# arkiven4/glow-tts

Hardware: AMD Instinct MI355X
Metric: mel_frames_per_sec_train_step (higher is better)
Workload: dtype bf16; 1 GPU; configs/base.json, LJSpeech-shaped synthetic batches, B=32/GPU, T_x<=150, T_y<=800, bf16 GEMMs; batch_per_gpu=32, T_x=150, T_y=800, batches_rotated=8, padded_frames_per_gpu_step=25600, rows_layout=ragged, graphs_captured=6, parallelism=dp1 (utterance-sharded, RCCL gradient all-reduce, fp32 on the wire), launch=one HIP graph per step (one per ragged-row bucket, captured up front)

## Files before the change

### glow-tts_amd/_lib.py

```python
import ctypes
import os

_HERE = os.path.dirname(os.path.abspath(__file__))
LIB_PATH = os.environ.get("GT_LIB") or os.path.join(_HERE, "libglowtts_hip.so")

c_void_p, c_int, c_i64, c_size_t, c_float, c_u32 = (ctypes.c_void_p, ctypes.c_int, ctypes.c_int64,
                                                    ctypes.c_size_t, ctypes.c_float, ctypes.c_uint32)


class Pointer(ctypes.c_void_p):

    @classmethod
    def from_param(cls, v):
        if hasattr(v, "data_ptr"):
            v = v.data_ptr()
        elif isinstance(v, ctypes.Structure):
            return ctypes.byref(v)
        return ctypes.c_void_p.from_param(v)


STATUS = "status"
c_void_p = Pointer

PROTOTYPES = {
    "gt_version": (ctypes.c_char_p, []),
    "gt_mas_f32": (STATUS, [c_void_p, c_void_p, c_void_p, c_void_p, c_void_p, c_int, c_void_p, c_void_p,
                            c_int, c_int, c_int, c_i64, c_i64, c_void_p, c_size_t, c_void_p, c_void_p]),
    "gt_mas_lds_bytes": (c_size_t, [c_int, c_int]),
    "gt_mas_workspace_bytes": (c_size_t, [c_int, c_int, c_int]),
    "gt_mas_long_f32": (STATUS, [c_void_p, c_void_p, c_void_p, c_void_p, c_void_p, c_int, c_void_p, c_void_p,
                                 c_int, c_int, c_int, c_i64, c_i64, c_void_p, c_size_t, c_void_p, c_void_p]),
    "gt_mas_long_workspace_bytes": (c_size_t, [c_int, c_int, c_int]),
    "gt_mas_lengths_from_mask_f32": (STATUS, [c_void_p, c_void_p, c_void_p, c_int, c_int, c_int,
                                              c_i64, c_i64, c_void_p]),
    "gt_conv_gemm_bf16": (STATUS, [c_void_p, c_int, c_void_p, c_void_p, c_void_p, c_int, c_void_p,
                                   c_void_p, c_int, c_int, c_void_p, c_int, c_void_p, c_void_p, c_int,
                                   c_int, c_int, c_int, c_int, c_int, c_int, c_int,
                                   c_int, c_int, c_float, c_u32, c_void_p, c_void_p, c_int, c_int, c_void_p]),
    "gt_conv_wgrad_workspace_bytes": (c_size_t, [c_int, c_int, c_int, c_int, c_void_p]),
    "gt_conv_wgrad_ci_tile": (c_int, [c_int]),
    "gt_conv_wgrad_bf16": (STATUS, [c_void_p, c_int, c_void_p, c_int, c_int, c_int, c_int, c_int, c_void_p, c_size_t, c_void_p]),
    "gt_weightnorm_bwd": (STATUS, [c_void_p, c_int, c_void_p, c_void_p, c_void_p, c_void_p, c_void_p, c_void_p,
                                   c_int, c_int, c_int, c_int, c_void_p]),
    "gt_conv_wgrad_batched": (STATUS, [c_void_p, c_void_p, c_int, c_int, c_int, c_void_p]),
    "gt_weightnorm_bwd_batched": (STATUS, [c_void_p, c_int, c_int, c_int, c_void_p]),
    "gt_adamw_flat": (STATUS, [c_void_p, c_void_p, c_void_p, c_void_p, c_size_t, c_void_p, c_void_p, c_void_p]),
    "gt_colsum": (STATUS, [c_void_p, c_int, c_int, c_void_p, c_int, c_int, c_void_p]),
    "gt_squeeze_rows_f32": (STATUS, [c_void_p, c_void_p, c_void_p, c_int, c_int, c_int, c_int, c_void_p, c_void_p]),
    "gt_unsqueeze_rows_f32": (STATUS, [c_void_p, c_void_p, c_void_p, c_int, c_int, c_int, c_int, c_void_p, c_void_p]),
    "gt_flow_scalars": (STATUS, [c_void_p, c_int, c_void_p, c_void_p, c_void_p]),
    "gt_flow_scalars_multi": (STATUS, [c_void_p, c_void_p, c_int, c_void_p, c_int, c_void_p]),
    "gt_actnorm_ddi": (STATUS, [c_void_p, c_void_p, c_int, c_int, c_int, c_void_p, c_void_p, c_void_p, c_void_p]),
    "gt_actnorm_invconv_fwd": (STATUS, [c_void_p, c_void_p, c_void_p, c_int, c_void_p, c_void_p, c_void_p, c_void_p,
                                        c_void_p, c_void_p, c_void_p, c_int, c_int, c_int, c_void_p]),
    "gt_actnorm_invconv_bwd": (STATUS, [c_void_p, c_void_p, c_void_p, c_void_p, c_void_p, c_void_p, c_void_p, c_void_p,
                                        c_void_p, c_void_p, c_void_p, c_void_p, c_void_p, c_int, c_int, c_int, c_void_p]),
    "gt_actnorm_invconv_rev": (STATUS, [c_void_p, c_void_p, c_void_p, c_int, c_void_p, c_void_p, c_void_p, c_void_p, c_int, c_int, c_void_p]),
    "gt_coupling_rev": (STATUS, [c_void_p, c_void_p, c_void_p, c_void_p, c_int, c_int, c_int, c_void_p]),
    "gt_coupling_fwd": (STATUS, [c_void_p, c_void_p, c_void_p, c_void_p, c_void_p, c_int, c_int, c_int, c_int, c_void_p, c_int, c_void_p]),
    "gt_coupling_bwd": (STATUS, [c_void_p, c_void_p, c_void_p, c_void_p, c_void_p, c_void_p, c_void_p,
                                 c_int, c_int, c_int, c_int, c_void_p, c_int, c_void_p]),
    "gt_gate_bwd": (STATUS, [c_void_p, c_int, c_void_p, c_void_p, c_int, c_void_p, c_int, c_void_p,
                             c_int, c_int, c_float, c_u32, c_void_p, c_void_p]),
    "gt_relu_drop_bwd": (STATUS, [c_void_p, c_int, c_void_p, c_int, c_void_p, c_int, c_int, c_int, c_float, c_void_p]),
    "gt_rows_add_bf16": (STATUS, [c_void_p, c_int, c_void_p, c_int, c_int, c_int, c_void_p]),
    "gt_rows_f32_to_bf16": (STATUS, [c_void_p, c_int, c_void_p, c_int, c_void_p, c_int, c_int, c_void_p]),
    "gt_layernorm_fwd": (STATUS, [c_void_p, c_void_p, c_int, c_void_p, c_void_p, c_void_p, c_void_p, c_void_p, c_int,
                                  c_void_p, c_void_p, c_int, c_int, c_float, c_float, c_u32, c_float, c_u32, c_int, c_void_p, c_void_p]),
    "gt_layernorm_bwd": (STATUS, [c_void_p, c_void_p, c_int, c_void_p, c_void_p, c_void_p, c_void_p, c_void_p, c_int, c_int,
                                  c_float, c_float, c_u32, c_float, c_u32, c_int, c_void_p, c_void_p, c_void_p, c_int,
                                  c_void_p, c_void_p, c_int, c_void_p, c_void_p, c_void_p]),
    "gt_layernorm_bwd_partial_rows": (c_int, [c_int]),
    "gt_layernorm_bwd_partials": (STATUS, [c_void_p, c_void_p, c_int, c_void_p, c_void_p, c_void_p, c_void_p, c_void_p, c_int, c_int,
                                           c_float, c_float, c_u32, c_float, c_u32, c_int, c_void_p, c_void_p, c_void_p, c_int,
                                           c_void_p, c_void_p, c_int, c_void_p, c_void_p]),
    "gt_param_partials_reduce": (STATUS, [c_void_p, c_void_p]),
    "gt_dds_bwd_partial_rows": (c_int, [c_int]),
    "gt_attn_fwd": (STATUS, [c_void_p, c_void_p, c_void_p, c_int, c_void_p, c_void_p, c_void_p, c_void_p, c_int, c_void_p,
                             c_int, c_int, c_int, c_void_p, c_int, c_int, c_int, c_float, c_u32, c_void_p, c_void_p]),
    "gt_attn_bwd_workspace_bytes": (c_size_t, [c_int, c_int, c_int]),
    "gt_attn_mfma_shape": (c_int, [c_int, c_int, c_int]),
    "gt_attn_long_shape": (c_int, [c_int, c_int, c_int]),
    "gt_attn_bwd": (STATUS, [c_void_p, c_void_p, c_void_p, c_int, c_void_p, c_void_p, c_void_p, c_void_p, c_int, c_void_p,
                             c_void_p, c_size_t, c_void_p, c_void_p, c_void_p, c_int, c_void_p, c_void_p,
                             c_int, c_int, c_int, c_void_p, c_int, c_int, c_int, c_float, c_u32, c_void_p, c_void_p]),
    "gt_attn_stats_bytes": (c_size_t, [c_int, c_int, c_int]),
    "gt_attn_bwd_stats_workspace_bytes": (c_size_t, [c_int, c_int, c_int]),
    "gt_attn_fwd_stats": (STATUS, [c_void_p, c_void_p, c_void_p, c_int, c_void_p, c_void_p, c_void_p, c_void_p, c_int, c_void_p,
                                   c_int, c_int, c_int, c_void_p, c_int, c_int, c_int, c_float, c_u32, c_void_p, c_void_p]),
    "gt_attn_bwd_stats": (STATUS, [c_void_p, c_void_p, c_void_p, c_int, c_void_p, c_void_p, c_void_p, c_void_p, c_int, c_void_p,
                                   c_void_p, c_size_t, c_void_p, c_void_p, c_void_p, c_int, c_void_p, c_void_p,
                                   c_int, c_int, c_int, c_void_p, c_int, c_int, c_int, c_float, c_u32, c_void_p, c_void_p]),
    "gt_embedding_fwd": (STATUS, [c_void_p, c_void_p, c_void_p, c_void_p, c_void_p, c_int, c_int, c_int, c_void_p, c_int, c_int, c_int, c_float, c_void_p]),
    "gt_embedding_bwd": (STATUS, [c_void_p, c_void_p, c_void_p, c_void_p, c_int, c_int, c_int, c_void_p, c_int, c_int, c_int, c_float, c_void_p]),
    "gt_rows_add_cond": (STATUS, [c_void_p, c_int, c_void_p, c_int, c_void_p, c_void_p, c_void_p, c_int, c_void_p, c_int,
                                  c_int, c_int, c_int, c_int, c_void_p, c_void_p]),
    "gt_rows_ctx_fill": (STATUS, [c_void_p, c_void_p, c_void_p, c_void_p, c_void_p, c_void_p, c_int, c_int, c_void_p]),
    "gt_step_inputs": (STATUS, [c_void_p, c_void_p]),
# ... 390 lines not shown
```

### glow-tts_amd/csrc/conv_wgrad.hip

```cpp
#include <stdlib.h>
#include "common.h"
#include "internal.h"
#include "mfma_frag.h"
#include "../../include/glowtts_hip.h"

namespace {

constexpr int SLAB_Q = 64;

typedef __attribute__((__vector_size__(4 * sizeof(short)))) short s16x4_t;

__device__ __forceinline__ unsigned lds_off(const void* p) { return (unsigned)reinterpret_cast<uintptr_t>(p); }

__device__ __forceinline__ bf16x8_t tr_frag(const unsigned char* p0, const unsigned char* p1) {
  const s16x4_t lo = __builtin_amdgcn_ds_read_tr16_b64_v4i16((__attribute__((address_space(3))) s16x4_t*)(uintptr_t)p0);
  const s16x4_t hi = __builtin_amdgcn_ds_read_tr16_b64_v4i16((__attribute__((address_space(3))) s16x4_t*)(uintptr_t)p1);
  typedef __attribute__((__vector_size__(8 * sizeof(short)))) short s16x8_t;
  s16x8_t v = {lo[0], lo[1], lo[2], lo[3], hi[0], hi[1], hi[2], hi[3]};
  return __builtin_bit_cast(bf16x8_t, v);
}

__device__ __forceinline__ void glds16(const void* src, unsigned dst_base) {
  unsigned keep;
  asm volatile("s_mov_b32 %0, m0\n\ts_mov_b32 m0, %2\n\ts_nop 0\n\t"
               "global_load_lds_dwordx4 %1, off\n\ts_mov_b32 m0, %0"
               : "=&s"(keep) : "v"(src), "s"(dst_base) : "memory");
}
template <int N> __device__ __forceinline__ void wait_vm() { asm volatile("s_waitcnt vmcnt(%0)" :: "n"(N) : "memory"); }

template <int TAPS, int NJ, int KB_, int NST_> struct WgGeo {
  static constexpr int KB = KB_, NST = NST_;
  static constexpr int XR = KB + TAPS - 1;
  static constexpr int XCH = 8 * NJ;
  static constexpr int YB = KB * 256, XB = XR * XCH * 16, STAGE = YB + XB;
  static constexpr int YI = KB / 16;
  static constexpr int NWX = XR * XCH / 4;
  static constexpr int XI = (NWX + 63) / 64;
  static constexpr int NLD = YI + XI;
  static constexpr int NB = TAPS * NJ;
  static constexpr int LDS = NST * STAGE;
  static_assert(KB % 16 == 0 && SLAB_Q % KB == 0, "stage rows");
  static_assert((XR * XCH) % 4 == 0, "X chunks split evenly over the waves");
  static_assert(LDS <= 80 * 1024, "two workgroups per CU");
  static_assert((NST - 2) * NLD <= 63, "vmcnt field");
  static_assert(TAPS == 1 || NJ == 1, "taps or channel groups");
};

template <int TAPS, int NJ, int KB_, int NST_>
__device__ __forceinline__ void wgrad_tile(
    const bf16_t* __restrict__ X, int ldx, const bf16_t* __restrict__ dY, int ldy,
    float* __restrict__ part, float* __restrict__ part_bias, int R, int Cin, int Cout, int slab_rows,
    int co0, int ci0, int slab, int co_begin, int Ncols)
{
  using G = WgGeo<TAPS, NJ, KB_, NST_>;
  constexpr int KB = G::KB, NST = G::NST, NB = G::NB;
  extern __shared__ __attribute__((aligned(1024))) unsigned char ring[];
  const int tid = threadIdx.x, lane = tid & 63, wave = __builtin_amdgcn_readfirstlane(tid >> 6);
  constexpr int padl = TAPS >> 1;
  const int mbeg = slab * slab_rows;
  const int mend = min(R, mbeg + slab_rows);
  const int nst = (mend - mbeg + KB - 1) / KB;
  const int wco = wave >> 1, wci = wave & 1;
  const bool do_bias = (ci0 == 0) && part_bias && wci == 0;

  f32x16_t acc[NB][2];
  float bsum[2] = {0.f, 0.f};
#pragma unroll
  for (int t = 0; t < NB; ++t)
#pragma unroll
    for (int j = 0; j < 2; ++j)
#pragma unroll
      for (int e = 0; e < 16; ++e) acc[t][j][e] = 0.0f;

  int yrow[G::YI], ycol[G::YI], xrow[G::XI], xcol[G::XI];
  bool xact[G::XI];
#pragma unroll
  for (int j = 0; j < G::YI; ++j) {
    const int L = j * 256 + tid, r = L >> 4, c = (L & 15) ^ ((r & 3) << 2);
    yrow[j] = r; ycol[j] = min(co0 + c * 8, Ncols - 8);
// ... 114 lines not shown
      const int ci = ci0 + j * 64 + wci * 32 + r;
#pragma unroll
      for (int i = 0; i < 2; ++i) {
        if (ci >= Cin) continue;
#pragma unroll
        for (int e = 0; e < 16; ++e) {
          const int co = co0 + wco * 64 + i * 32 + (e & 3) + 8 * (e >> 2) + 4 * h;
          if (co < Ncols) part[(((size_t)slab * TAPS + t) * Cout + co_begin + co) * Cin + ci] = acc[t * NJ + j][i][e];
        }
      }
    }
  if (do_bias) {
#pragma unroll
    for (int i = 0; i < 2; ++i) {
      const float tot = bsum[i] + __shfl_xor(bsum[i], 32);
      const int co = co0 + wco * 64 + i * 32 + r;
      if (h == 0 && co < Ncols) part_bias[(size_t)slab * Cout + co_begin + co] = tot;
    }
  }
}

template <int TAPS> struct WgSel;
template <> struct WgSel<5> { static constexpr int NJ = 1, KB = 64, NST = 3; };
template <> struct WgSel<3> { static constexpr int NJ = 1, KB = 64, NST = 3; };
template <> struct WgSel<1> { static constexpr int NJ = 3, KB = 32, NST = 3; };
template <int TAPS> using WgGeoT = WgGeo<TAPS, WgSel<TAPS>::NJ, WgSel<TAPS>::KB, WgSel<TAPS>::NST>;

template <int TAPS>
__global__ __launch_bounds__(256, 2) void gt_conv_wgrad_kernel(
    const bf16_t* __restrict__ X, int ldx, const bf16_t* __restrict__ dY, int ldy,
    float* __restrict__ part, float* __restrict__ part_bias, int R, int Cin, int Cout, int slab_rows)
{
  using S = WgSel<TAPS>;
  wgrad_tile<TAPS, S::NJ, S::KB, S::NST>(X, ldx, dY, ldy, part, part_bias, R, Cin, Cout, slab_rows,
                                         blockIdx.x * 128, blockIdx.y * 64 * S::NJ, blockIdx.z, 0, Cout);
}

template <int TAPS>
__global__ __launch_bounds__(256, 2) void gt_conv_wgrad_batched_kernel(
    const gt_wgrad_job* __restrict__ jobs, const gt_wgrad_tile* __restrict__ tiles)
{
  using S = WgSel<TAPS>;
  const gt_wgrad_tile t = tiles[blockIdx.x];
  const gt_wgrad_job j = jobs[t.job];
  wgrad_tile<TAPS, S::NJ, S::KB, S::NST>(static_cast<const bf16_t*>(j.X), j.ldx, static_cast<const bf16_t*>(j.dY), j.ldy,
                                         j.part, j.part_bias, j.R, j.Cin, j.Cout, j.slab_rows, t.co0, t.ci0, t.slab, j.co_begin, j.co_count);
}

template <int TAPS> static int wgrad_lds_attr()
{
  if (gt_allow_lds<&gt_conv_wgrad_kernel<TAPS>>(WgGeoT<TAPS>::LDS) || gt_allow_lds<&gt_conv_wgrad_batched_kernel<TAPS>>(WgGeoT<TAPS>::LDS)) return GT_E_LAUNCH;
  return 0;
}

constexpr int WNB_ROWS = 4;
__device__ __forceinline__ void weightnorm_bwd_row(
    const float* __restrict__ part, const float* __restrict__ part_bias, int S, const float* __restrict__ v,
    const float* __restrict__ g, const float* __restrict__ inv_norm, float* __restrict__ dv, float* __restrict__ dg,
    float* __restrict__ dbias, int Cout, int Cin, int taps, int accumulate, int co, float* dws)
{
  const int lane = threadIdx.x & 63, n = Cin * taps;
  if (dbias && lane == 0) {
    float sb = 0.f;
    for (int k = 0; k < S; ++k) sb += part_bias[(size_t)k * Cout + co];
    dbias[co] = accumulate ? dbias[co] + sb : sb;
  }
  const size_t sstride = (size_t)taps * Cout * Cin;
  for (int tap = 0; tap < taps; ++tap) {
    const float* pt = part + ((size_t)tap * Cout + co) * Cin;
    for (int ci = lane; ci < Cin; ci += 64) {
      const float* pp = pt + ci;
      float s0 = 0.f, s1 = 0.f, s2 = 0.f, s3 = 0.f;
      int k = 0;
      for (; k + 4 <= S; k += 4) {
        const float a0 = pp[(size_t)k * sstride], a1 = pp[(size_t)(k + 1) * sstride];
        const float a2 = pp[(size_t)(k + 2) * sstride], a3 = pp[(size_t)(k + 3) * sstride];
        s0 += a0; s1 += a1; s2 += a2; s3 += a3;
      }
      for (; k < S; ++k) s0 += pp[(size_t)k * sstride];
      dws[ci * taps + tap] = (s0 + s1) + (s2 + s3);
    }
  }
  __builtin_amdgcn_fence(__ATOMIC_RELEASE, "wavefront");
  __builtin_amdgcn_wave_barrier();
  __builtin_amdgcn_fence(__ATOMIC_ACQUIRE, "wavefront");
  const float* vr = v + (size_t)co * n;
  float* dr = dv + (size_t)co * n;
  if (!g) {
    for (int i = lane; i < n; i += 64) dr[i] = accumulate ? dr[i] + dws[i] : dws[i];
    return;
  }
  float dot = 0.f;
  for (int i = lane; i < n; i += 64) dot += dws[i] * vr[i];
  const float d = wave_sum(dot);
  const float inv = inv_norm[co], gg = g[co];
  if (lane == 0) dg[co] = accumulate ? dg[co] + d * inv : d * inv;
  const float a = gg * inv, bcoef = gg * d * inv * inv * inv;
  for (int i = lane; i < n; i += 64) {
    const float val = a * dws[i] - bcoef * vr[i];
    dr[i] = accumulate ? dr[i] + val : val;
  }
}

constexpr int WNF_P = 4;
typedef float wnf4_t __attribute__((ext_vector_type(4)));
__device__ __forceinline__ wnf4_t wnf_ld4(const float* p) { return *(const __attribute__((address_space(1))) wnf4_t*)(uintptr_t)p; }
// ... 244 lines not shown
                                  int taps, void* workspace, size_t workspace_bytes, void* stream)
{
  if (R <= 0 || Cin <= 0 || Cout <= 0) return GT_E_INVAL;
  if (!X || !dY || !workspace) return GT_E_INVAL;
  if (taps != 1 && taps != 3 && taps != 5) return GT_E_UNSUPPORTED;
  if ((Cin & 7) || (Cout & 7) || (ldx & 7) || (ldy & 7)) return GT_E_ALIGN;
  if (((uintptr_t)X | (uintptr_t)dY) & 15) return GT_E_ALIGN;
  int S = 0;
  if (workspace_bytes < gt_conv_wgrad_workspace_bytes(R, Cin, Cout, taps, &S)) return GT_E_INVAL;
  const int slab_rows = (((R + S - 1) / S) + SLAB_Q - 1) / SLAB_Q * SLAB_Q;
  const int cit = gt_conv_wgrad_ci_tile(taps);
  const dim3 grid((Cout + 127) / 128, (Cin + cit - 1) / cit, S);
  hipStream_t st = static_cast<hipStream_t>(stream);
  const bf16_t* x = static_cast<const bf16_t*>(X); const bf16_t* dy = static_cast<const bf16_t*>(dY);
  float* part = static_cast<float*>(workspace);
  float* pb = part + (size_t)S * taps * Cout * Cin;
  if (wgrad_lds_attr<5>() || wgrad_lds_attr<3>() || wgrad_lds_attr<1>()) return GT_E_LAUNCH;
  if (taps == 5)      hipLaunchKernelGGL(gt_conv_wgrad_kernel<5>, grid, dim3(256), WgGeoT<5>::LDS, st, x, ldx, dy, ldy, part, pb, R, Cin, Cout, slab_rows);
  else if (taps == 3) hipLaunchKernelGGL(gt_conv_wgrad_kernel<3>, grid, dim3(256), WgGeoT<3>::LDS, st, x, ldx, dy, ldy, part, pb, R, Cin, Cout, slab_rows);
  else                hipLaunchKernelGGL(gt_conv_wgrad_kernel<1>, grid, dim3(256), WgGeoT<1>::LDS, st, x, ldx, dy, ldy, part, pb, R, Cin, Cout, slab_rows);
  return gt_launch_status(__func__);
}

extern "C" int gt_weightnorm_bwd(const void* workspace, int R, const float* v, const float* g, const float* inv_norm,
                                 float* dv, float* dg, float* dbias, int Cout, int Cin, int taps, int accumulate, void* stream)
{
  if (!workspace || !v || !dv || Cout <= 0 || Cin <= 0 || taps <= 0) return GT_E_INVAL;
  if (g && (!inv_norm || !dg)) return GT_E_INVAL;
  int S = 0;
  gt_conv_wgrad_workspace_bytes(R, Cin, Cout, taps, &S);
  if ((size_t)WNB_ROWS * Cin * taps * sizeof(float) > WNB_LDS_MAX) return GT_E_UNSUPPORTED;
  const int rows = wnb_rows(Cin * taps);
  const size_t lds = wnb_lds(rows, Cin * taps);
  const float* part = static_cast<const float*>(workspace);
  hipLaunchKernelGGL(gt_weightnorm_bwd_kernel, dim3((Cout + rows - 1) / rows), dim3(64 * rows), lds, static_cast<hipStream_t>(stream),
                     part, part + (size_t)S * taps * Cout * Cin, S, v, g, inv_norm, dv, dg, dbias, Cout, Cin, taps, accumulate);
  return gt_launch_status(__func__);
}

extern "C" int gt_conv_wgrad_batched(const void* jobs_device, const void* tiles_device, int n_tiles5, int n_tiles3,
                                     int n_tiles1, void* stream)
{
  if (!jobs_device || !tiles_device || n_tiles5 < 0 || n_tiles3 < 0 || n_tiles1 < 0) return GT_E_INVAL;
  hipStream_t st = static_cast<hipStream_t>(stream);
  const gt_wgrad_job* jobs = static_cast<const gt_wgrad_job*>(jobs_device);
  const gt_wgrad_tile* tiles = static_cast<const gt_wgrad_tile*>(tiles_device);
  if (wgrad_lds_attr<5>() || wgrad_lds_attr<3>() || wgrad_lds_attr<1>()) return GT_E_LAUNCH;
  if (n_tiles5) hipLaunchKernelGGL(gt_conv_wgrad_batched_kernel<5>, dim3(n_tiles5), dim3(256), WgGeoT<5>::LDS, st, jobs, tiles);
  if (n_tiles3) hipLaunchKernelGGL(gt_conv_wgrad_batched_kernel<3>, dim3(n_tiles3), dim3(256), WgGeoT<3>::LDS, st, jobs, tiles + n_tiles5);
  if (n_tiles1) hipLaunchKernelGGL(gt_conv_wgrad_batched_kernel<1>, dim3(n_tiles1), dim3(256), WgGeoT<1>::LDS, st, jobs, tiles + n_tiles5 + n_tiles3);
  return gt_launch_status(__func__);
}

extern "C" int gt_weightnorm_bwd_batched(const void* jobs_device, int n_jobs, int total_rows, int max_row_elems, void* stream)
{
  if (!jobs_device || n_jobs <= 0 || total_rows <= 0 || max_row_elems <= 0) return GT_E_INVAL;
  if ((size_t)WNB_ROWS * max_row_elems * sizeof(float) > WNB_LDS_MAX) return GT_E_UNSUPPORTED;
  const int rows = wnb_rows(max_row_elems);
  const size_t lds = wnb_lds(rows, max_row_elems);
  hipLaunchKernelGGL(gt_weightnorm_bwd_batched_kernel, dim3((total_rows + rows - 1) / rows), dim3(64 * rows), lds,
                     static_cast<hipStream_t>(stream), static_cast<const gt_wnb_job*>(jobs_device), n_jobs, total_rows, max_row_elems);
  return gt_launch_status(__func__);
}

extern "C" int gt_colsum(const void* Y, int ldy, int is_f32, float* out, int R, int N, void* stream)
{
  if (!Y || !out || R < 0 || N <= 0) return GT_E_INVAL;
  if (R == 0) return GT_OK;
  const int rows_per_block = 128;
  const dim3 grid((N + 63) / 64, (R + rows_per_block - 1) / rows_per_block);
  hipStream_t st = static_cast<hipStream_t>(stream);
  if (is_f32) hipLaunchKernelGGL(gt_colsum_kernel<true>,  grid, dim3(256), 0, st, Y, ldy, out, R, N, rows_per_block);
  else        hipLaunchKernelGGL(gt_colsum_kernel<false>, grid, dim3(256), 0, st, Y, ldy, out, R, N, rows_per_block);
  return gt_launch_status(__func__);
}
```

### glow-tts_amd/wgrad.py

```python
import contextlib
import os
import types

import numpy as np
import torch

from . import _lib, devstate
from ._lib import call

JOB = np.dtype([("X", "u8"), ("dY", "u8"), ("part", "u8"), ("part_bias", "u8"), ("ldx", "i4"), ("ldy", "i4"), ("R", "i4"),
                ("Cin", "i4"), ("Cout", "i4"), ("co_begin", "i4"), ("co_count", "i4"), ("slab_rows", "i4")])
TILE = np.dtype([("job", "i4"), ("co0", "i4"), ("ci0", "i4"), ("slab", "i4")])
WNB = np.dtype([("part", "u8"), ("part_bias", "u8"), ("v", "u8"), ("g", "u8"), ("inv_norm", "u8"), ("dv", "u8"), ("dg", "u8"),
                ("dbias", "u8"), ("S", "i4"), ("Cout", "i4"), ("Cin", "i4"), ("taps", "i4"), ("row_start", "i4"),
                ("accumulate", "i4"), ("pad0_", "i4"), ("pad1_", "i4")])
assert JOB.itemsize == 64 and TILE.itemsize == 16 and WNB.itemsize == 96
C_STRUCTS = {"gt_wgrad_job": JOB, "gt_wgrad_tile": TILE, "gt_wnb_job": WNB}

SLOTS = 512
ROW_US = float(os.environ.get("GT_WGRAD_ROW_US", "0.033"))
WG_US = 3.0
PART_BPS = 2.0e6
MAX_SLABS = 32
XCDS = 8
CI_TILE = {5: 64, 3: 64, 1: 192}
FORCE_SLABS = int(os.environ.get("GT_WGRAD_SLABS", "0"))

ASYNC = os.environ.get("GT_WGRAD_ASYNC", "0") != "0"
_ACTIVE = []
_KEEP = []
_SCOPE = None


_POOL = []
_POOL_N, _POOL_BYTES = 64, 1 << 18


def _fill_pool():
    while len(_POOL) < _POOL_N:
        _POOL.append(torch.empty(_POOL_BYTES, dtype=torch.uint8).pin_memory())


class CaptureKeep(list):

    def release(self):
        for obj in self:
            if isinstance(obj, torch.Tensor) and not obj.is_cuda and obj.numel() == _POOL_BYTES and obj.is_pinned() and len(_POOL) < 4 * _POOL_N:
                _POOL.append(obj)
        self.clear()


@contextlib.contextmanager
def capture_scope(dev, nbytes=8 << 20):
    global _SCOPE
    arena = torch.empty(nbytes, dtype=torch.uint8, device=dev)
    sc = _SCOPE = types.SimpleNamespace(dev=dev, arena=arena, off=0, uploads=[], keep=CaptureKeep([arena]))
    try:
        yield sc.keep
        assert not (arena.is_cuda and torch.cuda.is_current_stream_capturing())
        for dst, host in sc.uploads:
            dst.copy_(host, non_blocking=True)
        if sc.uploads and arena.is_cuda:
            torch.cuda.current_stream(dev).synchronize()
    except BaseException:
        sc.keep.release()
        raise
    finally:
        sc.uploads.clear()
        _SCOPE = None


def capture_keep(obj):
    if _SCOPE is not None:
        if not any(o is obj for o in _SCOPE.keep):
            _SCOPE.keep.append(obj)
        return True
    return False


def choose_slabs(base_tiles, R, part_bytes):
    if FORCE_SLABS:
        return FORCE_SLABS
    best, costs = None, []
    for S in range(1, max(1, min(MAX_SLABS, R // 128)) + 1):
        rounds = -(-base_tiles * S // SLOTS)
        rows = -(-(-(-R // S)) // 64) * 64
        cost = rounds * (rows * ROW_US + WG_US) + S * part_bytes / PART_BPS
        costs.append((cost, S))
        best = cost if best is None else min(best, cost)
    return min(S for cost, S in costs if cost <= 1.05 * best)


def single_slabs(R, Cin, Cout, taps):
    import ctypes
    S = ctypes.c_int(0)
    call.gt_conv_wgrad_workspace_bytes(R, Cin, Cout, taps, ctypes.byref(S))
    return S.value


def _side_stream(dev):
    return devstate.get(dev).stream("wgrad_side")


def join(dev):
    st = devstate.get(dev)
    if st.pending:
        torch.cuda.current_stream(dev).wait_stream(st.stream("wgrad_side"))
        st.pending = False


def active():
    return _ACTIVE[-1] if _ACTIVE else None


def _scratch(dev, nbytes):
    return devstate.get(dev).scratch("wgrad_flush", nbytes, per_stream=True)


def _grad_out(param):
    fg = getattr(param, "_gt_flat_grad", None)
    if fg is None:
        return torch.empty_like(param)
    buf, off = fg
    return buf[off:off + param.numel()].view_as(param)


class WgradQueue:

    def __init__(self, device, site=None, accumulate=False, side_stream=False):
        self.dev = device
        self.site = site
        self.items = []
        self.accumulate, self.force_side = accumulate, side_stream
        self.defer_to = None
        self.ln_jobs = []
        self.params_done = []

    def __enter__(self):
        _ACTIVE.append(self)
        return self

    def __exit__(self, et, ev, tb):
        _ACTIVE.pop()
# ... 106 lines not shown
            devstate.get(dev).pending = True
        else:
            self._flush()

    def _keep(self, obj):
        if capture_keep(obj):
            return
        if self.site is not None:
            lst = getattr(self.site, "_wgrad_keep", None)
            if lst is None:
                lst = []
                object.__setattr__(self.site, "_wgrad_keep", lst)
            lst.append(obj)
        else:
            _KEEP.append(obj)

    def _flush(self):
        dev = self.dev
        jobs, tiles, wnbs, rows, max_n, nbytes = self._plan()
        ws = _scratch(dev, nbytes)
        base = ws.data_ptr()
        capturing = torch.cuda.is_current_stream_capturing()

        def upload(arr):
            raw = arr.view(np.uint8).reshape(-1)
            if capturing:
                if not _POOL or raw.size > _POOL_BYTES:
                    raise RuntimeError("wgrad tables: no pinned staging buffer available inside graph capture "
                                       "(run one eager step first)")
                full = _POOL.pop()
                host = full[: raw.size]
                host.numpy()[:] = raw
                self._keep(full)
                sc = _SCOPE
                nb = (raw.size + 255) & ~255
                if sc is not None and sc.dev == dev and sc.off + nb <= sc.arena.numel():
                    dst = sc.arena[sc.off:sc.off + raw.size]
                    sc.off += nb
                    sc.uploads.append((dst, host))
                    return dst
                return host.to(dev, non_blocking=True)
            host = torch.from_numpy(raw).pin_memory()
            return host.to(dev, non_blocking=True)

        if capturing:
            cache = {}
        else:
            _fill_pool()
            cache = getattr(self.site, "_wgrad_tables", None) if self.site is not None else None
            if cache is None:
                cache = {}
                if self.site is not None:
                    object.__setattr__(self.site, "_wgrad_tables", cache)
        skey = tuple((t, tuple(x[2:] for x in tiles[t]), tuple(j[6:] for j in jobs)) for t in (5, 3, 1))
        if cache.get("skey") != skey:
            tl, counts = [], []
            for taps in (5, 3, 1):
                n = 0
                order = sorted(range(len(tiles[taps])), key=lambda i: -tiles[taps][i][0])
                queues = [[] for _ in range(XCDS)]
                for i in order:
                    _, jid, nco, nci, S = tiles[taps][i]
                    for sl in range(S):
                        q = min(queues, key=len)
                        q += [(jid, co * 128, ci * CI_TILE[taps], sl) for co in range(nco) for ci in range(nci)]
                flat = [q[pos] for pos in range(max(map(len, queues), default=0)) for q in queues if pos < len(q)]
                if flat:
                    t = np.zeros(len(flat), dtype=TILE)
                    a = np.array(flat, dtype=np.int64)
                    t["job"], t["co0"], t["ci0"], t["slab"] = a[:, 0], a[:, 1], a[:, 2], a[:, 3]
                    tl.append(t)
                    n = len(flat)
                counts.append(n)
            ta = np.concatenate(tl) if tl else np.zeros(1, dtype=TILE)
            cache["skey"], cache["tiles"], cache["counts"] = skey, upload(ta), counts
            cache["pkey"] = None
        pkey = (base, tuple(j[:4] for j in jobs), tuple(w[2:8] for w in wnbs), self.accumulate)
        if cache.get("pkey") != pkey:
            ja = np.array([(j[0], j[1], base + j[2], (base + j[3]) if j[3] >= 0 else 0) + j[4:] for j in jobs], dtype=JOB)
            wa = np.array([(base + w[0], base + w[1]) + w[2:] for w in wnbs], dtype=WNB)
            cache["pkey"], cache["jobs"], cache["wnb"] = pkey, upload(ja), upload(wa)
        counts = cache["counts"]
        st = _lib.current_stream(dev)
        assert all(call.gt_conv_wgrad_ci_tile(t) == w for t, w in CI_TILE.items()), "wgrad.CI_TILE does not match the library's tile widths"
        call.gt_conv_wgrad_batched(cache["jobs"], cache["tiles"], counts[0], counts[1], counts[2], st)
        call.gt_weightnorm_bwd_batched(cache["wnb"], len(wnbs), rows, max_n, st)
        if capturing:
            self._keep(cache)
        self.items = []
```

### include/glowtts_hip.h

```cpp
#ifndef GLOWTTS_HIP_H
#define GLOWTTS_HIP_H

#include <stddef.h>
#include <stdint.h>

#ifdef __cplusplus
extern "C" {
#endif

#define GT_OK            0
#define GT_E_INVAL      -1
#define GT_E_UNSUPPORTED -2
#define GT_E_ALIGN      -3
#define GT_E_LAUNCH     -4

#define GT_DT_F32  0
#define GT_DT_I32  1
#define GT_DT_F16  2
#define GT_DT_BF16 3
#define GT_DT_U8   4

#define GT_MAS_ST_TX_GT_TY   1
#define GT_MAS_ST_BAD_LEN    2

// ... 26 lines not shown

int gt_mas_lengths_from_mask_f32(const float* mask, int32_t* t_x, int32_t* t_y,
                                 int B, int T_x, int T_y, int64_t stride_b, int64_t stride_x,
                                 void* stream);

#define GT_HALO 2

#define GT_TILE_AUTO 0
#define GT_TILE_64x64 1
#define GT_TILE_64x128 2
#define GT_TILE_128x64 3
#define GT_TILE_128x128 4
#define GT_TILE_256x64 5
#define GT_TILE_64x64_TAPS 6
int gt_conv_gemm_bf16(const void* X, int ldx, const void* Wp, const float* bias,
                      const float* cond, int ldc, const float* rowmask,
                      void* Y, int ldy, int out_f32, const void* addend, int ldadd,
                      void* gate_t, void* gate_s, int ldts,
                      int R, int N, int Cin, int taps, int Tp, int Np, int Kp,
                      int relu, int gate, float drop_p, uint32_t drop_seed, const uint32_t* seed_dev,
                      const int32_t* row0, int B, int tile, void* stream);

int gt_pack_conv_weights(const float* v, const float* g, void* pack_fwd, void* pack_dgrad,
                         float* inv_norm, int Cout, int Cin, int taps,
                         int Np_fwd, int Kp_fwd, int Np_dgrad, int Kp_dgrad, int gate, void* stream);

typedef struct gt_pack_desc {
  const float* v; const float* g; void* pack_fwd; void* pack_dgrad; float* inv_norm;
  int32_t Cout, Cin, taps, Np_fwd, Kp_fwd, Np_dgrad, Kp_dgrad, gate, row_start, pad_;
} gt_pack_desc;
int gt_pack_conv_weights_multi(const void* descs_device, int n_convs, int total_rows, int group8, void* stream);

size_t gt_conv_wgrad_workspace_bytes(int R, int Cin, int Cout, int taps, int* slabs_out);
int gt_conv_wgrad_ci_tile(int taps);
int gt_conv_wgrad_bf16(const void* X, int ldx, const void* dY, int ldy, int R, int Cin, int Cout,
                       int taps, void* workspace, size_t workspace_bytes, void* stream);

int gt_weightnorm_bwd(const void* workspace, int R, const float* v, const float* g, const float* inv_norm,
                      float* dv, float* dg, float* dbias, int Cout, int Cin, int taps, int accumulate, void* stream);

typedef struct gt_wgrad_job {
  const void* X; const void* dY; float* part; float* part_bias;
  int32_t ldx, ldy, R, Cin, Cout, co_begin, co_count, slab_rows;
} gt_wgrad_job;
typedef struct gt_wgrad_tile { int32_t job, co0, ci0, slab; } gt_wgrad_tile;
typedef struct gt_wnb_job {
  const float* part; const float* part_bias; const float* v; const float* g; const float* inv_norm;
  float* dv; float* dg; float* dbias;
  int32_t S, Cout, Cin, taps, row_start, accumulate, pad0_, pad1_;
} gt_wnb_job;
int gt_conv_wgrad_batched(const void* jobs_device, const void* tiles_device, int n_tiles5, int n_tiles3,
                          int n_tiles1, void* stream);
int gt_weightnorm_bwd_batched(const void* jobs_device, int n_jobs, int total_rows, int max_row_elems, void* stream);

int gt_colsum(const void* Y, int ldy, int is_f32, float* out, int R, int N, void* stream);

int gt_squeeze_rows_f32(const float* y, float* rows, const int32_t* len_sq, int B, int C, int Ty, int Tp,
                        const int32_t* row0, void* stream);
int gt_unsqueeze_rows_f32(const float* rows, float* y, const int32_t* len_sq, int B, int C, int Ty, int Tp,
                          const int32_t* row0, void* stream);

int gt_actnorm_ddi(const float* x, const int32_t* len, int B, int R, int C, double* workspace, float* logs, float* bias,
                   void* stream);

int gt_flow_scalars(const float* logs, int C, const float* W, float* scal, void* stream);
int gt_flow_scalars_multi(const void* logs_ptrs, const void* w_ptrs, int C, float* scal, int n, void* stream);
int gt_actnorm_invconv_fwd(const float* x, float* y, void* y0_bf16, int ld0, const float* logs, const float* bias,
                           const float* W, const float* scal, const float* rowmask, const int32_t* len,
                           float* logdet, int B, int R, int C, void* stream);
int gt_actnorm_invconv_bwd(const float* x, const float* dy, float* dx, const float* logs, const float* bias,
                           const float* W, const float* scal, const float* rowmask, const int32_t* len,
                           const float* dlogdet, float* dlogs, float* dbias, float* dW, int B, int R, int C, void* stream);

int gt_coupling_fwd(const float* out, const float* x, float* z, const float* rowmask, float* logdet,
                    int B, int R, int C, int Tp, const int32_t* row0, int sigmoid_scale, void* stream);
int gt_coupling_bwd(const float* out, const float* x, const float* dz, const float* dlogdet, const float* rowmask,
                    float* dx, void* dout_bf16, int B, int R, int C, int Tp, const int32_t* row0, int sigmoid_scale,
                    void* stream);

int gt_gate_bwd(const void* dacts, int ldd, const void* T, const void* S, int ldts, void* dpre, int ldp, void* dpre_cond,
                int R, int half, float drop_p, uint32_t drop_seed, const uint32_t* seed_dev, void* stream);

int gt_relu_drop_bwd(const void* d, int ldd, const void* y, int ldy, void* dc, int ldc, int R, int n, float drop_p, void* stream);

int gt_rows_add_bf16(float* dx, int ldx, const void* add, int lda, int R, int n, void* stream);
int gt_rows_f32_to_bf16(const float* in, int ldi, void* out, int ldo, const float* rowmask, int R, int n, void* stream);

int gt_layernorm_fwd(const float* a, const void* y, int ldy, const float* gamma, const float* beta, const float* rowmask,
                     float* out_f32, void* out_bf16, int ldo, float* mean, float* rstd, int R, int C, float eps,
                     float p_in, uint32_t seed_in, float p_out, uint32_t seed_out, int relu, const uint32_t* seed_dev, void* stream);
int gt_layernorm_bwd(const float* a, const void* y, int ldy, const float* gamma, const float* beta, const float* rowmask,
                     const float* mean, const float* rstd, int R, int C, float eps,
                     float p_in, uint32_t seed_in, float p_out, uint32_t seed_out, int relu, const uint32_t* seed_dev,
                     const float* dout_f32, const void* dout_bf16, int lddo,
                     float* da, void* dy, int lddy, float* dgamma, float* dbeta, void* stream);
int gt_layernorm_bwd_partial_rows(int R);
int gt_layernorm_bwd_partials(const float* a, const void* y, int ldy, const float* gamma, const float* beta, const float* rowmask,
                              const float* mean, const float* rstd, int R, int C, float eps,
                              float p_in, uint32_t seed_in, float p_out, uint32_t seed_out, int relu, const uint32_t* seed_dev,
                              const float* dout_f32, const void* dout_bf16, int lddo,
                              float* da, void* dy, int lddy, float* partials, void* stream);
#define GT_PARTIALS_MAX 32
typedef struct gt_partials_job { const float* partials; float* dst_a; float* dst_b; int32_t n_rows, Ca, Cb, pad_; } gt_partials_job;
typedef struct gt_partials_args { gt_partials_job job[GT_PARTIALS_MAX]; int32_t n_jobs; } gt_partials_args;
int gt_param_partials_reduce(const gt_partials_args* args, void* stream);

// ... 348 lines not shown
```

Baseline: 4.838 million mel-frames/s.

## Add paired 512-thread wgrad kernel sharing dY or X tiles across two output tiles

```diff
diff --git a/glow-tts_amd/_lib.py b/glow-tts_amd/_lib.py
--- a/glow-tts_amd/_lib.py
+++ b/glow-tts_amd/_lib.py
@@ -44,6 +44,7 @@
                                    c_int, c_int, c_int, c_int, c_void_p]),
     "gt_conv_wgrad_batched": (STATUS, [c_void_p, c_void_p, c_int, c_int, c_int, c_void_p]),
     "gt_weightnorm_bwd_batched": (STATUS, [c_void_p, c_int, c_int, c_int, c_void_p]),
+    "gt_conv_wgrad_paired": (STATUS, [c_void_p, c_void_p, c_int, c_int, c_void_p]),
     "gt_adamw_flat": (STATUS, [c_void_p, c_void_p, c_void_p, c_void_p, c_size_t, c_void_p, c_void_p, c_void_p]),
     "gt_colsum": (STATUS, [c_void_p, c_int, c_int, c_void_p, c_int, c_int, c_void_p]),
     "gt_squeeze_rows_f32": (STATUS, [c_void_p, c_void_p, c_void_p, c_int, c_int, c_int, c_int, c_void_p, c_void_p]),
diff --git a/glow-tts_amd/csrc/conv_wgrad.hip b/glow-tts_amd/csrc/conv_wgrad.hip
--- a/glow-tts_amd/csrc/conv_wgrad.hip
+++ b/glow-tts_amd/csrc/conv_wgrad.hip
@@ -25,6 +25,12 @@
   asm volatile("s_mov_b32 %0, m0\n\ts_mov_b32 m0, %2\n\ts_nop 0\n\t"
                "global_load_lds_dwordx4 %1, off\n\ts_mov_b32 m0, %0"
                : "=&s"(keep) : "v"(src), "s"(dst_base) : "memory");
+}
+__device__ __forceinline__ void glds16s(const void* base, unsigned off, unsigned dst_base) {
+  unsigned keep;
+  asm volatile("s_nop 4\n\ts_mov_b32 %0, m0\n\ts_mov_b32 m0, %3\n\ts_nop 0\n\t"
+               "global_load_lds_dwordx4 %1, %2\n\ts_mov_b32 m0, %0"
+               : "=&s"(keep) : "v"(off), "s"(base), "s"(dst_base) : "memory");
 }
 template <int N> __device__ __forceinline__ void wait_vm() { asm volatile("s_waitcnt vmcnt(%0)" :: "n"(N) : "memory"); }
 
@@ -245,6 +251,223 @@
   if (gt_allow_lds<&gt_conv_wgrad_kernel<TAPS>>(WgGeoT<TAPS>::LDS) || gt_allow_lds<&gt_conv_wgrad_batched_kernel<TAPS>>(WgGeoT<TAPS>::LDS)) return GT_E_LAUNCH;
   return 0;
 }
+
+template <int TAPS, int KIND> struct WgGeo8 {
+  static constexpr int KB = 64, NST = KIND ? 3 : 4;
+  static constexpr int NY = KIND ? 2 : 1;
+  static constexpr int XR = KB + TAPS - 1;
+  static constexpr int XCH = KIND ? 8 : 16;
+  static constexpr int YB = NY * KB * 256, XB = XR * XCH * 16, STAGE = YB + XB;
+  static constexpr int YI = NY * KB * 16 / 512;
+  static constexpr int NWX = XR * XCH / 8;
+  static constexpr int XI = (NWX + 63) / 64;
+  static constexpr int NLD = YI + XI;
+  static constexpr int LDS = NST * STAGE;
+  static_assert((XR * XCH) % 8 == 0, "X chunks split evenly over the waves");
+  static_assert(NWX > 64 * (XI - 1), "every wave issues all XI instructions");
+  static_assert(STAGE % 256 == 0 && YB % 256 == 0, "stages keep the bank phase");
+  static_assert(LDS <= 160 * 1024, "one workgroup per CU");
+  static_assert((NST - 2) * NLD <= 63, "vmcnt field");
+};
+
+template <int TAPS, int KIND>
+__device__ __forceinline__ void wgrad_pair_tile(
+    const bf16_t* __restrict__ X, int ldx, const bf16_t* __restrict__ dY, int ldy,
+    float* __restrict__ part, float* __restrict__ part_bias, int R, int Cin, int Cout, int slab_rows,
+    int co0, int ci0, int slab, int co_begin, int Ncols)
+{
+  using G = WgGeo8<TAPS, KIND>;
+  constexpr int KB = G::KB, NST = G::NST, NB = TAPS;
+  extern __shared__ __attribute__((aligned(1024))) unsigned char ring[];
+  const int tid = threadIdx.x, lane = tid & 63, wave = __builtin_amdgcn_readfirstlane(tid >> 6);
+  constexpr int padl = TAPS >> 1;
+  const int mbeg = slab * slab_rows;
+  const int mend = min(R, mbeg + slab_rows);
+  const int nst = (mend - mbeg + KB - 1) / KB;
+  const int grp = wave >> 2, wco = (wave >> 1) & 1, wci = wave & 1;
+  const int gco0 = co0 + (KIND ? grp * 128 : 0), gci0 = ci0 + (KIND ? 0 : grp * 64);
+  const bool live = KIND ? gco0 < Ncols : gci0 < Cin;
+  const bool do_bias = live && (gci0 == 0) && part_bias;
+
+  f32x16_t acc[NB][2];
+  float bsum = 0.f;
+#pragma unroll
+  for (int t = 0; t < NB; ++t)
+#pragma unroll
+    for (int j = 0; j < 2; ++j)
+#pragma unroll
+      for (int e = 0; e < 16; ++e) acc[t][j][e] = 0.0f;
+
+  int yrow[G::YI], ycol[G::YI], xrow[G::XI], xcol[G::XI];
+  bool xact[G::XI];
+#pragma unroll
+  for (int j = 0; j < G::YI; ++j) {
+    const int L = j * 512 + tid, r = (L >> 4) & 63, c = (L & 15) ^ ((r & 3) << 2);
+    yrow[j] = r; ycol[j] = min(co0 + (L >> 10) * 128 + c * 8, Ncols - 8);
+  }
+#pragma unroll
+  for (int j = 0; j < G::XI; ++j) {
+    const int Lw = j * 64 + lane, L = wave * G::NWX + Lw, r = L / G::XCH, cc = L - r * G::XCH;
+    const int c = KIND ? cc ^ (((r >> 1) & 1) << 2) : cc ^ ((r & 3) << 2);
+    xact[j] = Lw < G::NWX;
+    xrow[j] = r - padl; xcol[j] = min(ci0 + c * 8, Cin - 8);
+  }
+  const unsigned ring0 = lds_off(ring);
+  unsigned yoff[G::YI], xoff[G::XI];
+#pragma unroll
+  for (int j = 0; j < G::YI; ++j) yoff[j] = (unsigned)(yrow[j] * ldy + ycol[j]) * 2u;
+#pragma unroll
+  for (int j = 0; j < G::XI; ++j) xoff[j] = (unsigned)((xrow[j] + padl) * ldx + xcol[j]) * 2u;
+
+  auto issue = [&](int s, int sl_i) {
+    const int mb = mbeg + s * KB;
+    const unsigned slot = ring0 + (unsigned)sl_i * G::STAGE;
+    const bool edge = (mb - padl < 0) || (mb + KB + padl > R) || (mb + KB > mend);
+    if (!edge) {
+      const bf16_t* ys = dY + (size_t)mb * ldy;
+      const bf16_t* xs = X + (size_t)(mb - padl) * ldx;
+#pragma unroll
+      for (int j = 0; j < G::YI; ++j) glds16s(ys, yoff[j], slot + (unsigned)(j * 512 + wave * 64) * 16);
+#pragma unroll
+      for (int j = 0; j < G::XI; ++j)
+        if (xact[j]) glds16s(xs, xoff[j], slot + G::YB + (unsigned)(wave * G::NWX + j * 64) * 16);
+    } else {
+      unsigned char* sl = ring + (size_t)sl_i * G::STAGE;
+#pragma unroll
+      for (int j = 0; j < G::YI; ++j) {
+        const int m = mb + yrow[j];
+        u32x4_t v = {0u, 0u, 0u, 0u};
+        if (m < mend) v = *reinterpret_cast<const u32x4_t*>(dY + (size_t)m * ldy + ycol[j]);
+        *reinterpret_cast<u32x4_t*>(sl + (size_t)(j * 512 + tid) * 16) = v;
+      }
+#pragma unroll
+      for (int j = 0; j < G::XI; ++j) {
+        const int m = mb + xrow[j];
+        u32x4_t v = {0u, 0u, 0u, 0u};
+        if (xact[j]) {
+          if (m >= 0 && m < R) v = *reinterpret_cast<const u32x4_t*>(X + (size_t)m * ldx + xcol[j]);
+          *reinterpret_cast<u32x4_t*>(sl + G::YB + (size_t)(wave * G::NWX + j * 64 + lane) * 16) = v;
+        }
+      }
+    }
+  };
+
+  const int li = lane & 15, q = li >> 2, p = li & 3;
+  const int colhalf = ((lane >> 4) & 1) * 16;
+  const int h = lane >> 5;
+  constexpr int NOX = TAPS < 4 ? TAPS : 4;
+  int offA[2], offX[NOX];
+#pragma unroll
+  for (int i = 0; i < 2; ++i) {
+    const int ch = wco * 8 + i * 4 + (colhalf >> 3) + (p >> 1);
+    offA[i] = (KIND ? grp * KB * 256 : 0) + (8 * h + q) * 256 + ((ch ^ (q << 2)) << 4) + (p & 1) * 8;
+  }
+#pragma unroll
+  for (int t = 0; t < NOX; ++t) {
+    const int ch = (KIND ? 0 : grp * 8) + wci * 4 + (colhalf >> 3) + (p >> 1);
+    const int sw = KIND ? (((q + t) >> 1) & 1) << 2 : ((q + t) & 3) << 2;
+    offX[t] = (8 * h + q) * (G::XCH * 16) + ((ch ^ sw) << 4) + (p & 1) * 8;
+  }
+
+  bf16x8_t af[2][2], bfg[NB];
+  auto read_a = [&](int buf, const unsigned char* yb, int ks) {
+#pragma unroll
+    for (int i = 0; i < 2; ++i) {
+      const unsigned char* ya = yb + offA[i] + ks * 16 * 256;
+      af[buf][i] = tr_frag(ya, ya + 4 * 256);
+    }
+  };
+  auto read_b = [&](int t, const unsigned char* xb, int ks) {
+    const unsigned char* xa = xb + offX[t & 3] + (ks * 16 + t) * (G::XCH * 16);
+    bfg[t] = tr_frag(xa, xa + 4 * (G::XCH * 16));
+  };
+  auto kstep = [&](int ks, const unsigned char* ybn, const unsigned char* xbn, int ksn) {
+    const int cur = ks & 1;
+    read_a(cur ^ 1, ybn, ksn);
+    __builtin_amdgcn_sched_barrier(0);
+#pragma unroll
+    for (int t = 0; t < NB; ++t) {
+#pragma unroll
+      for (int i = 0; i < 2; ++i) acc[t][i] = __builtin_amdgcn_mfma_f32_32x32x16_bf16(af[cur][i], bfg[t], acc[t][i], 0, 0, 0);
+      read_b(t, xbn, ksn);
+      __builtin_amdgcn_sched_barrier(0);
+    }
+    if (do_bias) {
+      const u32x4_t w4 = __builtin_bit_cast(u32x4_t, wci ? af[cur][1] : af[cur][0]);
+#pragma unroll
+      for (int d = 0; d < 4; ++d) bsum += __uint_as_float(w4[d] << 16) + __uint_as_float(w4[d] & 0xffff0000u);
+    }
+  };
+
+#pragma unroll 1
+  for (int s = 0; s < NST - 1 && s < nst; ++s) issue(s, s);
+  int cslot = 0, islot = NST - 1;
+  int pend_s = -1, pend_slot = 0;
+  auto advance = [&](int s) {
+    const int after = min(nst - 1, s + NST - 2) - s;
+    if (after >= NST - 2) wait_vm<(NST - 2) * G::NLD>();
+    else wait_vm<0>();
+    asm volatile("s_waitcnt lgkmcnt(0)\n\ts_barrier" ::: "memory");
+    if (s + NST - 1 < nst) {
+      if (grp == 0) issue(s + NST - 1, islot);
+      else { pend_s = s + NST - 1; pend_slot = islot; }
+    }
+    islot = islot + 1 == NST ? 0 : islot + 1;
+  };
+  advance(0);
+  const unsigned char* yb = ring;
+  if (live) {
+    read_a(0, yb, 0);
+#pragma unroll
+    for (int t = 0; t < NB; ++t) read_b(t, yb + G::YB, 0);
+  }
+#pragma unroll 1
+  for (int s = 0; s < nst; ++s) {
+    if (live) {
+#pragma unroll
+      for (int ks = 0; ks < KB / 16 - 1; ++ks) kstep(ks, yb, yb + G::YB, ks + 1);
+    }
+    if (pend_s >= 0) { issue(pend_s, pend_slot); pend_s = -1; }
+    if (s + 1 < nst) advance(s + 1);
+    cslot = cslot + 1 == NST ? 0 : cslot + 1;
+    yb = ring + (size_t)cslot * G::STAGE;
+    if (live) kstep(KB / 16 - 1, yb, yb + G::YB, 0);
+  }
+  if (!live) return;
+
+  const int r = lane & 31;
+#pragma unroll
+  for (int t = 0; t < TAPS; ++t) {
+    const int ci = gci0 + wci * 32 + r;
+#pragma unroll
+    for (int i = 0; i < 2; ++i) {
+      if (ci >= Cin) continue;
+#pragma unroll
+      for (int e = 0; e < 16; ++e) {
+        const int co = gco0 + wco * 64 + i * 32 + (e & 3) + 8 * (e >> 2) + 4 * h;
+        if (co < Ncols) part[(((size_t)slab * TAPS + t) * Cout + co_begin + co) * Cin + ci] = acc[t][i][e];
+      }
+    }
+  }
+  if (do_bias) {
+    const float tot = bsum + __shfl_xor(bsum, 32);
+    const int co = gco0 + wco * 64 + wci * 32 + r;
+    if (h == 0 && co < Ncols) part_bias[(size_t)slab * Cout + co_begin + co] = tot;
+  }
+}
+
+template <int TAPS>
+__global__ __launch_bounds__(512, 1) void gt_conv_wgrad_paired_kernel(
+    const gt_wgrad_job* __restrict__ jobs, const gt_wgrad_pair* __restrict__ pairs)
+{
+  const gt_wgrad_pair t = pairs[blockIdx.x];
+  const gt_wgrad_job j = jobs[t.job];
+  const bf16_t* x = static_cast<const bf16_t*>(j.X); const bf16_t* dy = static_cast<const bf16_t*>(j.dY);
+  if (t.kind == 0) wgrad_pair_tile<TAPS, 0>(x, j.ldx, dy, j.ldy, j.part, j.part_bias, j.R, j.Cin, j.Cout, j.slab_rows, t.co0, t.ci0, t.slab, j.co_begin, j.co_count);
+  else             wgrad_pair_tile<TAPS, 1>(x, j.ldx, dy, j.ldy, j.part, j.part_bias, j.R, j.Cin, j.Cout, j.slab_rows, t.co0, t.ci0, t.slab, j.co_begin, j.co_count);
+}
+
+template <int TAPS> constexpr int wgrad_pair_lds() { return WgGeo8<TAPS, 0>::LDS > WgGeo8<TAPS, 1>::LDS ? WgGeo8<TAPS, 0>::LDS : WgGeo8<TAPS, 1>::LDS; }
 
 constexpr int WNB_ROWS = 4;
 __device__ __forceinline__ void weightnorm_bwd_row(
@@ -595,6 +818,18 @@
   return gt_launch_status(__func__);
 }
 
+extern "C" int gt_conv_wgrad_paired(const void* jobs_device, const void* pairs_device, int n_pairs5, int n_pairs3, void* stream)
+{
+  if (!jobs_device || !pairs_device || n_pairs5 < 0 || n_pairs3 < 0) return GT_E_INVAL;
+  hipStream_t st = static_cast<hipStream_t>(stream);
+  const gt_wgrad_job* jobs = static_cast<const gt_wgrad_job*>(jobs_device);
+  const gt_wgrad_pair* pairs = static_cast<const gt_wgrad_pair*>(pairs_device);
+  if (gt_allow_lds<&gt_conv_wgrad_paired_kernel<5>>(wgrad_pair_lds<5>()) || gt_allow_lds<&gt_conv_wgrad_paired_kernel<3>>(wgrad_pair_lds<3>())) return GT_E_LAUNCH;
+  if (n_pairs5) hipLaunchKernelGGL(gt_conv_wgrad_paired_kernel<5>, dim3(n_pairs5), dim3(512), wgrad_pair_lds<5>(), st, jobs, pairs);
+  if (n_pairs3) hipLaunchKernelGGL(gt_conv_wgrad_paired_kernel<3>, dim3(n_pairs3), dim3(512), wgrad_pair_lds<3>(), st, jobs, pairs + n_pairs5);
+  return gt_launch_status(__func__);
+}
+
 extern "C" int gt_weightnorm_bwd_batched(const void* jobs_device, int n_jobs, int total_rows, int max_row_elems, void* stream)
 {
   if (!jobs_device || n_jobs <= 0 || total_rows <= 0 || max_row_elems <= 0) return GT_E_INVAL;
diff --git a/glow-tts_amd/wgrad.py b/glow-tts_amd/wgrad.py
--- a/glow-tts_amd/wgrad.py
+++ b/glow-tts_amd/wgrad.py
@@ -14,8 +14,9 @@
 WNB = np.dtype([("part", "u8"), ("part_bias", "u8"), ("v", "u8"), ("g", "u8"), ("inv_norm", "u8"), ("dv", "u8"), ("dg", "u8"),
                 ("dbias", "u8"), ("S", "i4"), ("Cout", "i4"), ("Cin", "i4"), ("taps", "i4"), ("row_start", "i4"),
                 ("accumulate", "i4"), ("pad0_", "i4"), ("pad1_", "i4")])
-assert JOB.itemsize == 64 and TILE.itemsize == 16 and WNB.itemsize == 96
-C_STRUCTS = {"gt_wgrad_job": JOB, "gt_wgrad_tile": TILE, "gt_wnb_job": WNB}
+PAIR = np.dtype([("job", "i4"), ("co0", "i4"), ("ci0", "i4"), ("slab", "i4"), ("kind", "i4"), ("pad0_", "i4"), ("pad1_", "i4"), ("pad2_", "i4")])
+assert JOB.itemsize == 64 and TILE.itemsize == 16 and WNB.itemsize == 96 and PAIR.itemsize == 32
+C_STRUCTS = {"gt_wgrad_job": JOB, "gt_wgrad_tile": TILE, "gt_wnb_job": WNB, "gt_wgrad_pair": PAIR}
 
 SLOTS = 512
 ROW_US = float(os.environ.get("GT_WGRAD_ROW_US", "0.033"))
@@ -25,6 +26,8 @@
 XCDS = 8
 CI_TILE = {5: 64, 3: 64, 1: 192}
 FORCE_SLABS = int(os.environ.get("GT_WGRAD_SLABS", "0"))
+PAIRED = os.environ.get("GT_WGRAD_PAIRED", "1") != "0"
+PAIR_MIN_WGS = int(os.environ.get("GT_WGRAD_PAIR_MIN", "128"))
 
 ASYNC = os.environ.get("GT_WGRAD_ASYNC", "0") != "0"
 _ACTIVE = []
@@ -89,6 +92,15 @@
         costs.append((cost, S))
         best = cost if best is None else min(best, cost)
     return min(S for cost, S in costs if cost <= 1.05 * best)
+
+
+def pair_grid(nco, nci):
+    out = [(co, ci, 0) for co in range(nco) for ci in range(0, nci - 1, 2)]
+    if nci & 1:
+        out += [(co, nci - 1, 1) for co in range(0, nco - 1, 2)]
+        if nco & 1:
+            out.append((nco - 1, nci - 1, 0))
+    return out
 
 
 def single_slabs(R, Cin, Cout, taps):
@@ -301,37 +313,48 @@
                 cache = {}
                 if self.site is not None:
                     object.__setattr__(self.site, "_wgrad_tables", cache)
-        skey = tuple((t, tuple(x[2:] for x in tiles[t]), tuple(j[6:] for j in jobs)) for t in (5, 3, 1))
+        skey = tuple((t, tuple(x[2:] for x in tiles[t]), tuple(j[6:] for j in jobs)) for t in (5, 3, 1)) + (PAIRED, PAIR_MIN_WGS)
         if cache.get("skey") != skey:
-            tl, counts = [], []
+            tl, counts, pl, pcounts = [], [], [], []
             for taps in (5, 3, 1):
-                n = 0
                 order = sorted(range(len(tiles[taps])), key=lambda i: -tiles[taps][i][0])
+                paired = PAIRED and taps != 1 and sum(len(pair_grid(x[2], x[3])) * x[4] for x in tiles[taps]) >= PAIR_MIN_WGS
                 queues = [[] for _ in range(XCDS)]
                 for i in order:
                     _, jid, nco, nci, S = tiles[taps][i]
                     for sl in range(S):
                         q = min(queues, key=len)
-                        q += [(jid, co * 128, ci * CI_TILE[taps], sl) for co in range(nco) for ci in range(nci)]
+                        if paired:
+                            q += [(jid, co * 128, ci * CI_TILE[taps], sl, kind) for co, ci, kind in pair_grid(nco, nci)]
+                        else:
+                            q += [(jid, co * 128, ci * CI_TILE[taps], sl) for co in range(nco) for ci in range(nci)]
                 flat = [q[pos] for pos in range(max(map(len, queues), default=0)) for q in queues if pos < len(q)]
+                t = np.zeros(len(flat), dtype=PAIR if paired else TILE)
                 if flat:
-                    t = np.zeros(len(flat), dtype=TILE)
                     a = np.array(flat, dtype=np.int64)
                     t["job"], t["co0"], t["ci0"], t["slab"] = a[:, 0], a[:, 1], a[:, 2], a[:, 3]
-                    tl.append(t)
-                    n = len(flat)
-                counts.append(n)
-            ta = np.concatenate(tl) if tl else np.zeros(1, dtype=TILE)
-            cache["skey"], cache["tiles"], cache["counts"] = skey, upload(ta), counts
+                    if paired:
+                        t["kind"] = a[:, 4]
+                    (pl if paired else tl).append(t)
+                counts.append(0 if paired else len(flat))
+                if taps != 1:
+                    pcounts.append(len(flat) if paired else 0)
+            ta = (np.concatenate(tl) if tl else np.zeros(1, dtype=TILE)).view(np.uint8)
+            pair_off = (ta.size + 255) & ~255
+            if pl:
+                ta = np.concatenate([ta, np.zeros(pair_off - ta.size, dtype=np.uint8), np.concatenate(pl).view(np.uint8)])
+            cache["skey"], cache["tiles"], cache["counts"], cache["pcounts"], cache["pair_off"] = skey, upload(ta), counts, pcounts, pair_off
             cache["pkey"] = None
         pkey = (base, tuple(j[:4] for j in jobs), tuple(w[2:8] for w in wnbs), self.accumulate)
         if cache.get("pkey") != pkey:
             ja = np.array([(j[0], j[1], base + j[2], (base + j[3]) if j[3] >= 0 else 0) + j[4:] for j in jobs], dtype=JOB)
             wa = np.array([(base + w[0], base + w[1]) + w[2:] for w in wnbs], dtype=WNB)
             cache["pkey"], cache["jobs"], cache["wnb"] = pkey, upload(ja), upload(wa)
-        counts = cache["counts"]
+        counts, pcounts = cache["counts"], cache["pcounts"]
         st = _lib.current_stream(dev)
         assert all(call.gt_conv_wgrad_ci_tile(t) == w for t, w in CI_TILE.items()), "wgrad.CI_TILE does not match the library's tile widths"
+        if any(pcounts):
+            call.gt_conv_wgrad_paired(cache["jobs"], cache["tiles"][cache["pair_off"]:], pcounts[0], pcounts[1], st)
         call.gt_conv_wgrad_batched(cache["jobs"], cache["tiles"], counts[0], counts[1], counts[2], st)
         call.gt_weightnorm_bwd_batched(cache["wnb"], len(wnbs), rows, max_n, st)
         if capturing:
diff --git a/include/glowtts_hip.h b/include/glowtts_hip.h
--- a/include/glowtts_hip.h
+++ b/include/glowtts_hip.h
@@ -102,6 +102,9 @@
 int gt_conv_wgrad_batched(const void* jobs_device, const void* tiles_device, int n_tiles5, int n_tiles3,
                           int n_tiles1, void* stream);
 int gt_weightnorm_bwd_batched(const void* jobs_device, int n_jobs, int total_rows, int max_row_elems, void* stream);
+
+typedef struct gt_wgrad_pair { int32_t job, co0, ci0, slab, kind, pad0_, pad1_, pad2_; } gt_wgrad_pair;
+int gt_conv_wgrad_paired(const void* jobs_device, const void* pairs_device, int n_pairs5, int n_pairs3, void* stream);
 
 int gt_colsum(const void* Y, int ldy, int is_f32, float* out, int R, int N, void* stream);
 
```

Measured after the change: 4.904 million mel-frames/s, median of 6. 1.01x the previous value.
